# myscience/open-genie

Hardware: NVIDIA H100
Metric: videotokenizer_train_step_frames_per_sec (higher is better)
Workload: dtype bf16

## Files before the change

open_genie_b200/csrc/conv3d_igemm.cu:

```cuda
#include "og_host.cuh"
#include "og_ptx.cuh"

namespace og {
extern std::atomic<uint64_t> g_launches;

struct IgemmSeg {
  int cin_blocks;
  int n[3], tap0[3], tstep[3], sh0[3], shstep[3];
  int kh, kw;
};

struct IgemmParams {
  int nseg;
  IgemmSeg seg[2];
  int sx[3];
  int OT, OH, OW;
  int om[3], oo[3];
  int b_mn_major;
  int block_n;
  int num_n_tiles, num_m_tiles;
  int bw_log2, bh_log2, bt_log2, bn_log2;
  int tiles_w, tiles_h, tiles_t;
  int N, T, H, W;
  int n_out;
  long long ldo;
  void* out;
  int out_f32;
  int vec_ok;
  const float* bias0;
  const float* bias1;
  int num_stages;
  int num_kb;
  int fast_store;
  const __nv_bfloat16* residual;
  double* gn_sums;
  int splits;
  float* ws;
  long long ws_slab;
};


static constexpr int kBlockM = 128;
static constexpr int kBlockK = 64;
static constexpr int kABytes = kBlockM * kBlockK * 2;
static constexpr int kMaxStages = 8;
static constexpr int kThreads = 256;
static constexpr int kTailBytes = 256 + 1024 + 4 * 4096 + 256;
__host__ __device__ constexpr int acc_ld(int bn) { return bn + 4; }

template <int NV>
__device__ __forceinline__ void ld_acc_row(const float* src, uint32_t (&v)[32]) {
#pragma unroll
  for (int i = 0; i < NV / 4; ++i) {
    const float4 f = reinterpret_cast<const float4*>(src)[i];
    v[4 * i] = __float_as_uint(f.x);
    v[4 * i + 1] = __float_as_uint(f.y);
    v[4 * i + 2] = __float_as_uint(f.z);
    v[4 * i + 3] = __float_as_uint(f.w);
  }
#pragma unroll
  for (int i = NV; i < 32; ++i) v[i] = 0u;
}

struct TileCoord {
  int n0, t0, h0, w0;
};

__device__ __forceinline__ TileCoord decode_m_tile(const IgemmParams& p, int m_tile) {
  TileCoord c;
  int per_sample = p.tiles_w * p.tiles_h * p.tiles_t;
  const int tn = m_tile / per_sample;
  c.n0 = tn << p.bn_log2;
  int r = m_tile - tn * per_sample;
  int tw = r % p.tiles_w;
  r /= p.tiles_w;
  int th = r % p.tiles_h;
  int tt = r / p.tiles_h;
  c.w0 = tw << p.bw_log2;
  c.h0 = th << p.bh_log2;
  c.t0 = tt << p.bt_log2;
  return c;
}

template <int BN, int BMN>
__global__ void __launch_bounds__(kThreads, 1)
    og_conv_igemm_kernel(const __grid_constant__ CUtensorMap mapA0, const __grid_constant__ CUtensorMap mapA1,
                         const __grid_constant__ CUtensorMap mapB, const IgemmParams p) {
  extern __shared__ uint8_t smem_raw[];
  uint8_t* smem = reinterpret_cast<uint8_t*>((reinterpret_cast<uintptr_t>(smem_raw) + 1023) & ~uintptr_t(1023));
  const int b_bytes = p.block_n * kBlockK * 2;
  const int a_bytes = kABytes;
  const int stage_bytes = a_bytes + b_bytes;
  uint64_t* bars = reinterpret_cast<uint64_t*>(smem + p.num_stages * stage_bytes);
  uint64_t* full = bars;
  uint64_t* empty = bars + kMaxStages;
  float* bias_s = reinterpret_cast<float*>(bars + 32);
  uint8_t* stage_s = reinterpret_cast<uint8_t*>(bars + 32) + 1024;
  double* stat_s = reinterpret_cast<double*>(stage_s + 4 * 4096);
  float* acc_s = reinterpret_cast<float*>(reinterpret_cast<uint8_t*>(bars) + kTailBytes);

  const int warp = warp_idx_uniform();
  const int lane = threadIdx.x & 31;
  const int total_tiles = p.num_m_tiles * p.num_n_tiles * p.splits;

  if (warp == 0 && lane == 0) {
    tma_prefetch_desc(&mapA0);
    if (p.nseg > 1) tma_prefetch_desc(&mapA1);
    tma_prefetch_desc(&mapB);
    for (int s = 0; s < p.num_stages; ++s) {
      mbar_init(&full[s], 1);
      mbar_init(&empty[s], 4);
    }
    fence_mbar_init();
  }
  __syncthreads();

  if (warp == 0) {
    {
      int stage = 0;
      uint32_t phase = 0;
      for (int item = blockIdx.x; item < total_tiles; item += gridDim.x) {
        const int tile = item / p.splits, split = item - tile * p.splits;
        const int m_super = tile / p.num_n_tiles;
        const int n_tile = tile - m_super * p.num_n_tiles;
        const TileCoord tc = decode_m_tile(p, m_super);
        const int kb_begin = (int)(((long long)p.num_kb * split) / p.splits);
        const int kb_end = (int)(((long long)p.num_kb * (split + 1)) / p.splits);
        const int nkb0 = p.seg[0].cin_blocks * p.seg[0].n[0] * p.seg[0].n[1] * p.seg[0].n[2];
        int sidx = (kb_begin >= nkb0 && p.nseg > 1) ? 1 : 0;
        IgemmSeg sg = p.seg[sidx];
        int rel = kb_begin - (sidx ? nkb0 : 0);
        int tapc = rel / sg.cin_blocks;
        int cb = rel - tapc * sg.cin_blocks;
        int jt = tapc / (sg.n[1] * sg.n[2]);
        int jh = (tapc / sg.n[2]) % sg.n[1];
        int jw = tapc % sg.n[2];
        const int aw0 = tc.w0 * p.sx[2], ah0 = tc.h0 * p.sx[1], at0 = tc.t0 * p.sx[0];
        for (int kb = kb_begin; kb < kb_end; ++kb) {
          const CUtensorMap* mapA = (sidx == 0) ? &mapA0 : &mapA1;
          const int dt = sg.sh0[0] + jt * sg.shstep[0], dh = sg.sh0[1] + jh * sg.shstep[1],
                    dw = sg.sh0[2] + jw * sg.shstep[2];
          mbar_wait(&empty[stage], phase ^ 1);
          uint8_t* sa = smem + stage * stage_bytes;
          uint8_t* sb = sa + a_bytes;
          if (elect_one()) {
            mbar_expect_tx(&full[stage], (uint32_t)stage_bytes);
            tma_load_5d(sa, mapA, &full[stage], cb * kBlockK, aw0 + dw, ah0 + dh, at0 + dt, tc.n0);
            if (!BMN) {
              tma_load_2d(sb, &mapB, &full[stage], kb * kBlockK, n_tile * p.block_n);
            } else {
              const int tap = ((sg.tap0[0] + jt * sg.tstep[0]) * sg.kh + sg.tap0[1] + jh * sg.tstep[1]) * sg.kw +
                              sg.tap0[2] + jw * sg.tstep[2];
              for (int pp = 0; pp < p.block_n / 64; ++pp)
                tma_load_3d(sb + pp * (64 * 128), &mapB, &full[stage], n_tile * p.block_n + pp * 64, tap,
                            cb * kBlockK);
            }
          }
          __syncwarp();
          if (++stage == p.num_stages) {
            stage = 0;
            phase ^= 1;
          }
          if (++cb == sg.cin_blocks) {
            cb = 0;
            if (++jw == sg.n[2]) {
              jw = 0;
              if (++jh == sg.n[1]) {
                jh = 0;
                if (++jt == sg.n[0]) {
                  sidx = 1;
                  sg = p.seg[1];
                  jt = jh = jw = 0;
                }
              }
            }
          }
        }
      }
    }
  } else if (warp >= 4) {
    const int q = warp & 3;
    const int row = q * 32 + lane;
    const int et = threadIdx.x - 128;
    int stage = 0;
    uint32_t phase = 0;
    float fl_s = 0.f, fl_ss = 0.f;
    if (et == 0) stat_s[0] = stat_s[1] = 0.0;
    asm volatile("bar.sync 1, 128;" ::: "memory");
    for (int item = blockIdx.x; item < total_tiles; item += gridDim.x) {
      const int tile = item / p.splits;
      const int split = item - tile * p.splits;
      const int m_super = tile / p.num_n_tiles;
      const int n_tile = tile - m_super * p.num_n_tiles;
      const int nkb = (int)(((long long)p.num_kb * (split + 1)) / p.splits) -
                      (int)(((long long)p.num_kb * split) / p.splits);
      float acc[2][BN / 2];
#pragma unroll
      for (int hh = 0; hh < 2; ++hh)
#pragma unroll
        for (int i = 0; i < BN / 2; ++i) acc[hh][i] = 0.f;
      int prev = -1;
      for (int kb = 0; kb < nkb; ++kb) {
        mbar_wait(&full[stage], phase);
        const uint32_t a_addr = smem_u32(smem + stage * stage_bytes);
        const uint32_t b_addr = a_addr + a_bytes;
        wgmma_fence();
#pragma unroll
        for (int k = 0; k < kBlockK / 16; ++k) {
          const uint64_t bdesc = BMN ? gmma_desc_sw128(b_addr + k * 2048, 64 * 128, 1024)
                                     : gmma_desc_sw128(b_addr + k * 32, 16, 1024);
#pragma unroll
          for (int hh = 0; hh < 2; ++hh)
            wgmma_ss<BN, 0, BMN>(acc[hh], gmma_desc_sw128(a_addr + hh * 8192 + k * 32, 16, 1024), bdesc, 1);
        }
        wgmma_commit();
        wgmma_wait<1>();
        if (prev >= 0 && lane == 0) mbar_arrive(&empty[prev]);
        prev = stage;
        if (++stage == p.num_stages) {
          stage = 0;
          phase ^= 1;
        }
      }
      wgmma_wait<0>();
      reg_fence(acc[0]);
      reg_fence(acc[1]);
      if (prev >= 0 && lane == 0) mbar_arrive(&empty[prev]);
      asm volatile("bar.sync 1, 128;" ::: "memory");
      {
        const int r0 = q * 16 + (lane >> 2), c0 = 2 * (lane & 3);
#pragma unroll
        for (int hh = 0; hh < 2; ++hh)
#pragma unroll
          for (int j = 0; j < BN / 8; ++j) {
            float* d0 = acc_s + (hh * 64 + r0) * acc_ld(BN) + j * 8 + c0;
            *reinterpret_cast<float2*>(d0) = make_float2(acc[hh][4 * j], acc[hh][4 * j + 1]);
            *reinterpret_cast<float2*>(d0 + 8 * acc_ld(BN)) = make_float2(acc[hh][4 * j + 2], acc[hh][4 * j + 3]);
          }
      }
      asm volatile("bar.sync 1, 128;" ::: "memory");
      const float* acc_row = acc_s + row * acc_ld(BN);

      do {
      const TileCoord tc = decode_m_tile(p, m_super);
      const int dw = row & ((1 << p.bw_log2) - 1);
      const int dh = (row >> p.bw_log2) & ((1 << p.bh_log2) - 1);
      const int dt = (row >> (p.bw_log2 + p.bh_log2)) & ((1 << p.bt_log2) - 1);
      const int dn = row >> (p.bw_log2 + p.bh_log2 + p.bt_log2);
      const int vn = tc.n0 + dn, vt = tc.t0 + dt, vh = tc.h0 + dh, vw = tc.w0 + dw;
      const bool row_ok = vn < p.N && vt < p.T && vh < p.H && vw < p.W;
      const long long vox = (((long long)vn * p.OT + vt * p.om[0] + p.oo[0]) * p.OH + vh * p.om[1] + p.oo[1]) * p.OW +
                            vw * p.om[2] + p.oo[2];
      const int col0 = n_tile * p.block_n;

      if (p.splits > 1) {
        for (int c = 0; c < p.block_n; c += 32) {
          if (col0 + c >= p.n_out) break;
          uint32_t v[32];
          ld_acc_row<32>(acc_row + c, v);
          if (row_ok) {
            float* dst = p.ws + (long long)split * p.ws_slab + vox * p.ldo + col0 + c;
            if (p.vec_ok && col0 + c + 32 <= p.n_out) {
#pragma unroll
              for (int j = 0; j < 32; j += 4)
                __stcg(reinterpret_cast<float4*>(dst + j),
                       make_float4(__uint_as_float(v[j]), __uint_as_float(v[j + 1]), __uint_as_float(v[j + 2]),
                                   __uint_as_float(v[j + 3])));
            } else {
              for (int j = 0; j < 32; ++j)
                if (col0 + c + j < p.n_out) dst[j] = __uint_as_float(v[j]);
            }
          }
        }
        continue;
      }

      if (p.fast_store) {
        {
          asm volatile("bar.sync 1, 128;" ::: "memory");
          for (int j = et; j < p.block_n; j += 128) {
            const int col = col0 + j;
            float b = 0.f;
            if (col < p.n_out) {
              if (p.bias0) b += __ldg(p.bias0 + col);
              if (p.bias1) b += __ldg(p.bias1 + col);
            }
            bias_s[j] = b;
          }
          asm volatile("bar.sync 1, 128;" ::: "memory");
        }
        float st_s = 0.f, st_ss = 0.f;
        uint8_t* my_stage = stage_s + q * 4096;
        __nv_bfloat16* outp = reinterpret_cast<__nv_bfloat16*>(p.out);
        for (int c = 0; c < p.block_n; c += 64) {
          if (col0 + c >= p.n_out) break;
          uint32_t v0[32], v1[32];
          ld_acc_row<32>(acc_row + c, v0);
          ld_acc_row<32>(acc_row + c + 32, v1);
          if (p.residual && row_ok) {
            const uint4* rp = reinterpret_cast<const uint4*>(p.residual + vox * p.ldo + col0 + c);
#pragma unroll
            for (int j = 0; j < 8; ++j) {
              const uint4 u = __ldg(rp + j);
              const __nv_bfloat162* hh = reinterpret_cast<const __nv_bfloat162*>(&u);
#pragma unroll
              for (int e = 0; e < 4; ++e) {
                const float2 f = __bfloat1622float2(hh[e]);
                uint32_t* dst = (j < 4) ? &v0[8 * j + 2 * e] : &v1[8 * (j - 4) + 2 * e];
                dst[0] = __float_as_uint(__uint_as_float(dst[0]) + f.x);
                dst[1] = __float_as_uint(__uint_as_float(dst[1]) + f.y);
              }
            }
          }
#pragma unroll
          for (int j = 0; j < 32; ++j) {
            v0[j] = __float_as_uint(__uint_as_float(v0[j]) + bias_s[c + j]);
            v1[j] = __float_as_uint(__uint_as_float(v1[j]) + bias_s[c + 32 + j]);
          }
          if (p.gn_sums && row_ok) {
#pragma unroll
            for (int j = 0; j < 32; ++j) {
              const float r0 = __bfloat162float(__float2bfloat16_rn(__uint_as_float(v0[j])));
              const float r1 = __bfloat162float(__float2bfloat16_rn(__uint_as_float(v1[j])));
              st_s += r0 + r1;
              st_ss = fmaf(r0, r0, fmaf(r1, r1, st_ss));
            }
          }
#pragma unroll
          for (int j = 0; j < 4; ++j) {
            uint4 u;
            u.x = pack_bf16x2(__uint_as_float(v0[8 * j + 0]), __uint_as_float(v0[8 * j + 1]));
            u.y = pack_bf16x2(__uint_as_float(v0[8 * j + 2]), __uint_as_float(v0[8 * j + 3]));
            u.z = pack_bf16x2(__uint_as_float(v0[8 * j + 4]), __uint_as_float(v0[8 * j + 5]));
            u.w = pack_bf16x2(__uint_as_float(v0[8 * j + 6]), __uint_as_float(v0[8 * j + 7]));
            *reinterpret_cast<uint4*>(my_stage + lane * 128 + ((j ^ (lane & 7)) << 4)) = u;
          }
#pragma unroll
          for (int j = 0; j < 4; ++j) {
            uint4 u;
            u.x = pack_bf16x2(__uint_as_float(v1[8 * j + 0]), __uint_as_float(v1[8 * j + 1]));
            u.y = pack_bf16x2(__uint_as_float(v1[8 * j + 2]), __uint_as_float(v1[8 * j + 3]));
            u.z = pack_bf16x2(__uint_as_float(v1[8 * j + 4]), __uint_as_float(v1[8 * j + 5]));
            u.w = pack_bf16x2(__uint_as_float(v1[8 * j + 6]), __uint_as_float(v1[8 * j + 7]));
            *reinterpret_cast<uint4*>(my_stage + lane * 128 + (((j + 4) ^ (lane & 7)) << 4)) = u;
          }
          __syncwarp();
          const int chunk = lane & 7;
#pragma unroll
          for (int i = 0; i < 8; ++i) {
            const int r = i * 4 + (lane >> 3);
            const long long rvox = __shfl_sync(0xffffffffu, vox, r);
            const int rok = __shfl_sync(0xffffffffu, (int)row_ok, r);
            const uint4 u = *reinterpret_cast<const uint4*>(my_stage + r * 128 + ((chunk ^ (r & 7)) << 4));
            if (rok) *reinterpret_cast<uint4*>(outp + rvox * p.ldo + col0 + c + chunk * 8) = u;
          }
          __syncwarp();
        }
        fl_s += st_s;
        fl_ss += st_ss;
        continue;
      }

      for (int c = 0; c < p.block_n; c += 32) {
        uint32_t v[32];
        if (BN >= 32)
          ld_acc_row<32>(acc_row + c, v);
        else
          ld_acc_row<16>(acc_row + c, v);
        const int cbase = col0 + c;
        if (cbase >= p.n_out || !row_ok) continue;
        float f[32];
#pragma unroll
        for (int j = 0; j < 32; ++j) {
          float b = 0.f;
          const int col = cbase + j;
          if (col < p.n_out) {
            if (p.bias0) b += __ldg(p.bias0 + col);
            if (p.bias1) b += __ldg(p.bias1 + col);
          }
          f[j] = __uint_as_float(v[j]) + b;
          if (p.residual && col < p.n_out && row_ok) f[j] += __bfloat162float(p.residual[vox * p.ldo + col]);
        }
        if (p.out_f32) {
          float* o = reinterpret_cast<float*>(p.out) + vox * p.ldo + cbase;
          if (p.vec_ok && cbase + 32 <= p.n_out) {
#pragma unroll
            for (int j = 0; j < 32; j += 4)
              *reinterpret_cast<float4*>(o + j) = make_float4(f[j], f[j + 1], f[j + 2], f[j + 3]);
          } else {
            for (int j = 0; j < 32; ++j)
              if (cbase + j < p.n_out) o[j] = f[j];
          }
        } else {
          __nv_bfloat16* o = reinterpret_cast<__nv_bfloat16*>(p.out) + vox * p.ldo + cbase;
          if (p.vec_ok && cbase + 32 <= p.n_out) {
#pragma unroll
            for (int j = 0; j < 32; j += 8) {
              uint4 u;
              u.x = pack_bf16x2(f[j], f[j + 1]);
              u.y = pack_bf16x2(f[j + 2], f[j + 3]);
              u.z = pack_bf16x2(f[j + 4], f[j + 5]);
              u.w = pack_bf16x2(f[j + 6], f[j + 7]);
              *reinterpret_cast<uint4*>(o + j) = u;
            }
          } else {
            for (int j = 0; j < 32; ++j)
              if (cbase + j < p.n_out) o[j] = __float2bfloat16_rn(f[j]);
          }
        }
      }
      } while (0);
      if (p.fast_store && p.splits == 1 && p.gn_sums) {
        const TileCoord tcf = decode_m_tile(p, m_super);
        for (int o = 16; o > 0; o >>= 1) {
          fl_s += __shfl_xor_sync(0xffffffffu, fl_s, o);
          fl_ss += __shfl_xor_sync(0xffffffffu, fl_ss, o);
        }
        if (lane == 0) {
          atomicAdd(&stat_s[0], (double)fl_s);
          atomicAdd(&stat_s[1], (double)fl_ss);
        }
        asm volatile("bar.sync 1, 128;" ::: "memory");
        if (et == 0) {
          atomicAdd(&p.gn_sums[(long long)tcf.n0 * 2], stat_s[0]);
          atomicAdd(&p.gn_sums[(long long)tcf.n0 * 2 + 1], stat_s[1]);
          stat_s[0] = 0.0;
          stat_s[1] = 0.0;
        }
        fl_s = fl_ss = 0.f;
      }
    }
  }
}

template <int VEC>
__global__ void __launch_bounds__(256)
    og_splitk_finish_kernel(const float* __restrict__ ws, long long slab, int nslab, const float* __restrict__ bias0,
                            const float* __restrict__ bias1, void* __restrict__ out, int out_f32, int n_out,
                            long long per_sample, double* __restrict__ gn_sums) {
  const long long base = (long long)blockIdx.y * per_sample;
  float s = 0.f, ss = 0.f;
  for (long long i = ((long long)blockIdx.x * blockDim.x + threadIdx.x) * VEC; i < per_sample;
       i += (long long)gridDim.x * blockDim.x * VEC) {
    float v[VEC];
    if (VEC == 4) {
      const float4 a = __ldcg(reinterpret_cast<const float4*>(ws + base + i));
      v[0] = a.x; v[1 % VEC] = a.y; v[2 % VEC] = a.z; v[3 % VEC] = a.w;
      for (int k = 1; k < nslab; ++k) {
        const float4 b = __ldcg(reinterpret_cast<const float4*>(ws + (long long)k * slab + base + i));
        v[0] += b.x; v[1 % VEC] += b.y; v[2 % VEC] += b.z; v[3 % VEC] += b.w;
      }
    } else {
      v[0] = __ldcg(ws + base + i);
      for (int k = 1; k < nslab; ++k) v[0] += __ldcg(ws + (long long)k * slab + base + i);
    }
    const int col = (int)(i % n_out);
#pragma unroll
    for (int e = 0; e < VEC; ++e) {
      if (bias0) v[e] += __ldg(bias0 + col + e);
      if (bias1) v[e] += __ldg(bias1 + col + e);
    }
    if (out_f32) {
#pragma unroll
      for (int e = 0; e < VEC; ++e) reinterpret_cast<float*>(out)[base + i + e] = v[e];
    } else {
      __nv_bfloat16 h[VEC];
#pragma unroll
      for (int e = 0; e < VEC; ++e) {
        h[e] = __float2bfloat16_rn(v[e]);
        const float r = __bfloat162float(h[e]);
        s += r;
        ss = fmaf(r, r, ss);
      }
      __nv_bfloat16* o = reinterpret_cast<__nv_bfloat16*>(out) + base + i;
      if (VEC == 4)
        *reinterpret_cast<uint2*>(o) = *reinterpret_cast<const uint2*>(h);
      else
        o[0] = h[0];
    }
  }
  if (gn_sums) {
    __shared__ float red[2][8];
#pragma unroll
    for (int off = 16; off >= 1; off >>= 1) {
      s += __shfl_xor_sync(0xffffffffu, s, off);
      ss += __shfl_xor_sync(0xffffffffu, ss, off);
    }
    if ((threadIdx.x & 31) == 0) {
      red[0][threadIdx.x >> 5] = s;
      red[1][threadIdx.x >> 5] = ss;
    }
    __syncthreads();
    if (threadIdx.x == 0) {
      double a = 0.0, b = 0.0;
      for (int w = 0; w < (int)(blockDim.x >> 5); ++w) {
        a += (double)red[0][w];
        b += (double)red[1][w];
      }
      atomicAdd(gn_sums + 2 * blockIdx.y, a);
      atomicAdd(gn_sums + 2 * blockIdx.y + 1, b);
    }
  }
}

static int pick_block_n(int n_out, bool mn_major) {
  int bn = 16;
  while (bn < n_out && bn < 128) bn *= 2;
  if (mn_major && bn < 64) bn = 64;
  return bn;
}

template <int BN, int BMN>
static int launch_igemm_kernel(int grid, size_t smem_bytes, cudaStream_t stream, const CUtensorMap& mapA0,
                               const CUtensorMap& mapA1, const CUtensorMap& mapB, const IgemmParams& p) {
  static bool attr_set = false;
  if (!attr_set) {
    OG_CHECK_CUDA(cudaFuncSetAttribute(og_conv_igemm_kernel<BN, BMN>, cudaFuncAttributeMaxDynamicSharedMemorySize,
                                       227 * 1024));
    attr_set = true;
  }
  og_conv_igemm_kernel<BN, BMN><<<grid, kThreads, smem_bytes, stream>>>(mapA0, mapA1, mapB, p);
  OG_CHECK_CUDA(cudaGetLastError());
  return OG_OK;
}

struct IgemmLaunch {
  const void* a0 = nullptr;
  int c0 = 0;
  int aT = 0, aH = 0, aW = 0;
  int astride[3] = {1, 1, 1};
  const void* a1 = nullptr;
  int c1 = 0;
  IgemmSeg segs[2];
  int nseg = 1;
  const void* w = nullptr;
  int ldw = 0, k_off = 0, b_mn_major = 0, b_rows = 0, b_ntaps = 0;
  const float* bias0 = nullptr;
  const float* bias1 = nullptr;
  const void* residual = nullptr;
  void* out = nullptr;
  int out_f32 = 0;
  int N = 0, T = 0, H = 0, W = 0;
  int OT = 0, OH = 0, OW = 0;
  int om[3] = {1, 1, 1}, oo[3] = {0, 0, 0};
  int n_out = 0;
  void* workspace = nullptr;
  size_t workspace_bytes = 0;
  double* gn_sums = nullptr;
};

static IgemmSeg make_seg(int cin_blocks, int kt, int kh, int kw, int pt, int ph, int pw, int sgn) {
  IgemmSeg g;
  g.cin_blocks = cin_blocks;
  const int k[3] = {kt, kh, kw}, pd[3] = {pt, ph, pw};
  for (int d = 0; d < 3; ++d) {
    g.n[d] = k[d];
    g.tap0[d] = 0;
    g.tstep[d] = 1;
    g.sh0[d] = -sgn * pd[d];
    g.shstep[d] = sgn;
  }
  g.kh = kh;
  g.kw = kw;
  return g;
}

static int launch_igemm(const IgemmLaunch& L, cudaStream_t stream) {
  const int N = L.N, T = L.T, H = L.H, W = L.W, n_out = L.n_out;
  OG_REQUIRE(N > 0 && T > 0 && H > 0 && W > 0 && n_out > 0, "conv3d: empty problem");
  const bool plain = (L.OT == 0) && L.astride[0] == 1 && L.astride[1] == 1 && L.astride[2] == 1;
  int bw, bh, bt, bn;
  choose_voxel_box(kBlockM, N, T, H, W, &bw, &bh, &bt, &bn);
  IgemmParams p;
  memset(&p, 0, sizeof(p));
  p.nseg = L.nseg;
  p.num_kb = 0;
  for (int s = 0; s < L.nseg; ++s) {
    p.seg[s] = L.segs[s];
    p.num_kb += L.segs[s].cin_blocks * L.segs[s].n[0] * L.segs[s].n[1] * L.segs[s].n[2];
  }
  OG_REQUIRE(p.num_kb > 0, "conv3d: empty reduction");
  for (int d = 0; d < 3; ++d) {
    p.sx[d] = L.astride[d];
    p.om[d] = L.om[d];
    p.oo[d] = L.oo[d];
  }
  p.OT = L.OT ? L.OT : T;
  p.OH = L.OH ? L.OH : H;
  p.OW = L.OW ? L.OW : W;
  p.b_mn_major = L.b_mn_major;
  p.bw_log2 = ilog2(bw);
  p.bh_log2 = ilog2(bh);
  p.bt_log2 = ilog2(bt);
  p.bn_log2 = ilog2(bn);
  p.tiles_w = (W + bw - 1) / bw;
  p.tiles_h = (H + bh - 1) / bh;
  p.tiles_t = (T + bt - 1) / bt;
  p.N = N;
  p.T = T;
  p.H = H;
  p.W = W;
  p.num_m_tiles = ((N + bn - 1) / bn) * p.tiles_w * p.tiles_h * p.tiles_t;
  p.block_n = pick_block_n(n_out, L.b_mn_major != 0);
  p.num_n_tiles = (n_out + p.block_n - 1) / p.block_n;
  p.n_out = n_out;
  p.ldo = n_out;
  p.out = L.out;
  p.out_f32 = L.out_f32;
  p.vec_ok = L.out_f32 ? (n_out % 4 == 0) : (n_out % 8 == 0);
  p.bias0 = L.bias0;
  p.bias1 = L.bias1;
  p.residual = reinterpret_cast<const __nv_bfloat16*>(L.residual);
  const int stage_bytes = kABytes + p.block_n * kBlockK * 2;
  p.fast_store = (!L.out_f32 && n_out % 64 == 0 && p.block_n % 64 == 0) ? 1 : 0;
  p.splits = 1;
  if (plain) {
    const long long tiles = (long long)p.num_m_tiles * p.num_n_tiles;
    const size_t need = (size_t)N * T * H * W * n_out * sizeof(float);
    if (tiles * 2 <= num_sms() && p.num_kb >= 32 && L.workspace && !L.residual) {
      int sp = (int)(num_sms() / tiles);
      if (sp > p.num_kb / 8) sp = p.num_kb / 8;
      if (sp > 16) sp = 16;
      if ((size_t)sp > L.workspace_bytes / need) sp = (int)(L.workspace_bytes / need);
      if (sp >= 2) {
        p.splits = sp;
        p.ws = reinterpret_cast<float*>(L.workspace);
        p.ws_slab = (long long)(need / sizeof(float));
      }
    }
  }
  const int tail_bytes = kTailBytes + kBlockM * acc_ld(p.block_n) * 4 ;
  int stages = (227 * 1024 - 1024  - tail_bytes) / stage_bytes;
  if (stages > kMaxStages) stages = kMaxStages;
  p.num_stages = stages;
  const size_t smem_bytes = (size_t)stages * stage_bytes + 1024 + tail_bytes;

  CUtensorMap mapA0, mapA1, mapB;
  {
    const int c0 = L.c0;
    const int st = L.astride[0], sh = L.astride[1], sw = L.astride[2];
    uint64_t dims[5] = {(uint64_t)c0, (uint64_t)L.aW, (uint64_t)L.aH, (uint64_t)L.aT, (uint64_t)N};
    uint64_t str[4] = {(uint64_t)c0 * 2, (uint64_t)L.aW * c0 * 2, (uint64_t)L.aH * L.aW * c0 * 2,
                       (uint64_t)L.aT * L.aH * L.aW * c0 * 2};
    uint32_t box[5] = {kBlockK, (uint32_t)(bw * sw), (uint32_t)(bh * sh), (uint32_t)(bt * st), (uint32_t)bn};
    uint32_t es[5] = {1, (uint32_t)sw, (uint32_t)sh, (uint32_t)st, 1};
    OG_REQUIRE(box[1] <= 256 && box[2] <= 256 && box[3] <= 256, "conv3d: strided box exceeds the TMA limit");
    int r = make_tmap_bf16(&mapA0, L.a0, 5, dims, str, box, es);
    if (r != OG_OK) return r;
  }
  if (L.nseg > 1) {
    const int c1 = L.c1;
    uint64_t dims[5] = {(uint64_t)c1, (uint64_t)W, (uint64_t)H, (uint64_t)T, (uint64_t)N};
    uint64_t str[4] = {(uint64_t)c1 * 2, (uint64_t)W * c1 * 2, (uint64_t)H * W * c1 * 2, (uint64_t)T * H * W * c1 * 2};
    uint32_t box[5] = {kBlockK, (uint32_t)bw, (uint32_t)bh, (uint32_t)bt, (uint32_t)bn};
    int r = make_tmap_bf16(&mapA1, L.a1, 5, dims, str, box);
    if (r != OG_OK) return r;
  } else {
    mapA1 = mapA0;
  }
  const __nv_bfloat16* wb = reinterpret_cast<const __nv_bfloat16*>(L.w) + L.k_off;
  if (!L.b_mn_major) {
    uint64_t ktot = (uint64_t)p.num_kb * kBlockK;
    uint64_t dims[2] = {ktot, (uint64_t)n_out};
    uint64_t str[1] = {(uint64_t)L.ldw * 2};
    uint32_t box[2] = {kBlockK, (uint32_t)p.block_n};
    int r = make_tmap_bf16(&mapB, wb, 2, dims, str, box);
    if (r != OG_OK) return r;
  } else {
    uint64_t dims[3] = {(uint64_t)n_out, (uint64_t)L.b_ntaps, (uint64_t)L.b_rows};
    uint64_t str[2] = {(uint64_t)n_out * 2, (uint64_t)L.ldw * 2};
    uint32_t box[3] = {64, 1, 64};
    int r = make_tmap_bf16(&mapB, wb, 3, dims, str, box);
    if (r != OG_OK) return r;
  }

  const bool can_fuse = plain && p.fast_store && p.splits == 1 && bn == 1 && n_out <= 65536;
  p.gn_sums = (L.gn_sums && can_fuse) ? L.gn_sums : nullptr;
  const int total_tiles = p.num_m_tiles * p.num_n_tiles * p.splits;
  int grid = num_sms();
  if (grid > total_tiles) grid = total_tiles;
  int rc;
  switch (p.block_n * 2 + p.b_mn_major) {
    case 16 * 2: rc = launch_igemm_kernel<16, 0>(grid, smem_bytes, stream, mapA0, mapA1, mapB, p); break;
    case 32 * 2: rc = launch_igemm_kernel<32, 0>(grid, smem_bytes, stream, mapA0, mapA1, mapB, p); break;
    case 64 * 2: rc = launch_igemm_kernel<64, 0>(grid, smem_bytes, stream, mapA0, mapA1, mapB, p); break;
    case 128 * 2: rc = launch_igemm_kernel<128, 0>(grid, smem_bytes, stream, mapA0, mapA1, mapB, p); break;
    case 64 * 2 + 1: rc = launch_igemm_kernel<64, 1>(grid, smem_bytes, stream, mapA0, mapA1, mapB, p); break;
    case 128 * 2 + 1: rc = launch_igemm_kernel<128, 1>(grid, smem_bytes, stream, mapA0, mapA1, mapB, p); break;
    default: OG_REQUIRE(false, "conv3d: no kernel for block_n=%d", p.block_n);
  }
  if (rc != OG_OK) return rc;
  g_launches.fetch_add(1);
  bool finish_did_stats = false;
  if (p.splits > 1) {
    const long long per_sample = (long long)T * H * W * n_out;
    finish_did_stats = L.gn_sums && !L.out_f32;
    double* gs = finish_did_stats ? L.gn_sums : nullptr;
    const int vec = (n_out % 4 == 0) ? 4 : 1;
    long long bx = (per_sample / vec + 255) / 256;
    const long long cap = ((long long)num_sms() * 8 + N - 1) / N;
    if (bx > cap) bx = cap;
    if (bx < 1) bx = 1;
    dim3 grid((unsigned)bx, (unsigned)N);
    if (vec == 4)
      og_splitk_finish_kernel<4><<<grid, 256, 0, stream>>>(p.ws, p.ws_slab, p.splits, L.bias0, L.bias1, L.out, L.out_f32,
                                                            n_out, per_sample, gs);
    else
      og_splitk_finish_kernel<1><<<grid, 256, 0, stream>>>(p.ws, p.ws_slab, p.splits, L.bias0, L.bias1, L.out, L.out_f32,
                                                            n_out, per_sample, gs);
    OG_CHECK_CUDA(cudaGetLastError());
    g_launches.fetch_add(1);
  }
  if (L.gn_sums && !p.gn_sums && !finish_did_stats) {
    OG_REQUIRE(!L.out_f32 && plain, "conv3d: GroupNorm statistics need a plain bf16 output");
    int r = og_gn_stats(L.out, N, (int64_t)T * H * W, n_out, 1, L.gn_sums, (og_stream_t)stream);
    if (r != OG_OK) return r;
  }
  return OG_OK;
}

}

extern "C" int og_conv3d_fwd(const void* x0, int c0, int kt, int kh, int kw, int pt, int ph, int pw, const void* x1,
                             int c1, const void* w, int ldw, const float* bias0, const float* bias1,
                             const void* residual, void* out, int out_f32, int N, int T, int H, int W, int cout,
                             void* workspace, size_t workspace_bytes, double* gn_sums, og_stream_t stream) {
  using namespace og;
  OG_REQUIRE(x0 && w && out, "conv3d_fwd: null pointer");
  OG_REQUIRE(c0 > 0 && c0 % 64 == 0, "conv3d_fwd: c0=%d must be a positive multiple of 64", c0);
  OG_REQUIRE(!x1 || (c1 > 0 && c1 % 64 == 0), "conv3d_fwd: c1=%d must be a multiple of 64", c1);
  OG_REQUIRE(kt >= 1 && kh >= 1 && kw >= 1 && pt >= 0 && ph >= 0 && pw >= 0 && pt < kt && ph < kh && pw < kw,
             "conv3d_fwd: bad kernel/padding (%d,%d,%d)/(%d,%d,%d)", kt, kh, kw, pt, ph, pw);
  const int ktot = kt * kh * kw * c0 + (x1 ? c1 : 0);
  OG_REQUIRE(ldw >= ktot && ldw % 8 == 0, "conv3d_fwd: ldw=%d must be >= %d and a multiple of 8", ldw, ktot);
  IgemmLaunch L;
  L.a0 = x0; L.c0 = c0; L.aT = T; L.aH = H; L.aW = W;
  L.a1 = x1; L.c1 = c1;
  L.segs[0] = make_seg(c0 / 64, kt, kh, kw, pt, ph, pw, +1);
  L.segs[1] = make_seg(c1 / 64, 1, 1, 1, 0, 0, 0, +1);
  L.nseg = x1 ? 2 : 1;
  L.w = w; L.ldw = ldw;
  L.bias0 = bias0; L.bias1 = bias1; L.residual = residual;
  L.out = out; L.out_f32 = out_f32;
  L.N = N; L.T = T; L.H = H; L.W = W; L.n_out = cout;
  L.workspace = workspace; L.workspace_bytes = workspace_bytes;
  L.gn_sums = gn_sums;
  return launch_igemm(L, (cudaStream_t)stream);
}

extern "C" int og_conv3d_dgrad(const void* dy, int cout, int w_rows, const void* w, int ldw, int k_off, int kt, int kh,
                               int kw, int pt, int ph, int pw, void* dx, int dx_f32, int N, int T, int H, int W,
                               int cin, void* workspace, size_t workspace_bytes, og_stream_t stream) {
  using namespace og;
  OG_REQUIRE(dy && w && dx, "conv3d_dgrad: null pointer");
  OG_REQUIRE(cout > 0 && cout % 64 == 0, "conv3d_dgrad: cout=%d must be a multiple of 64", cout);
  OG_REQUIRE(cin > 0 && cin % 64 == 0, "conv3d_dgrad: cin=%d must be a multiple of 64", cin);
  OG_REQUIRE(k_off % 8 == 0 && ldw % 8 == 0, "conv3d_dgrad: k_off/ldw must be multiples of 8");
  OG_REQUIRE(w_rows > 0 && w_rows <= cout, "conv3d_dgrad: w_rows=%d must be in (0, cout]", w_rows);
  IgemmLaunch L;
  L.a0 = dy; L.c0 = cout; L.aT = T; L.aH = H; L.aW = W;
  L.segs[0] = make_seg(cout / 64, kt, kh, kw, pt, ph, pw, -1);
  L.nseg = 1;
  L.w = w; L.ldw = ldw; L.k_off = k_off; L.b_mn_major = 1; L.b_rows = w_rows; L.b_ntaps = kt * kh * kw;
  L.out = dx; L.out_f32 = dx_f32;
  L.N = N; L.T = T; L.H = H; L.W = W; L.n_out = cin;
  L.workspace = workspace; L.workspace_bytes = workspace_bytes;
  return launch_igemm(L, (cudaStream_t)stream);
}

static int out_extent(int in, int pad_front, int pad_back, int k, int s) { return (in + pad_front + pad_back - k) / s + 1; }

extern "C" int og_conv3d_strided_fwd(const void* x, int cin, int kt, int kh, int kw, int st, int sh, int sw, int pt, int ph,
                                     int pw, const void* w, int ldw, const float* bias, void* out, int out_f32, int N, int T,
                                     int H, int W, int cout, og_stream_t stream) {
  using namespace og;
  OG_REQUIRE(x && w && out, "conv3d_strided_fwd: null pointer");
  OG_REQUIRE(cin > 0 && cin % 64 == 0, "conv3d_strided_fwd: cin=%d must be a positive multiple of 64", cin);
  OG_REQUIRE(kt >= 1 && kh >= 1 && kw >= 1 && st >= 1 && sh >= 1 && sw >= 1 && st <= 8 && sh <= 8 && sw <= 8 && pt >= 0 &&
                 ph >= 0 && pw >= 0, "conv3d_strided_fwd: bad kernel / stride / padding");
  OG_REQUIRE(ldw >= kt * kh * kw * cin && ldw % 8 == 0, "conv3d_strided_fwd: bad ldw=%d", ldw);
  const int To = out_extent(T, pt, 0, kt, st), Ho = out_extent(H, ph, ph, kh, sh), Wo = out_extent(W, pw, pw, kw, sw);
  OG_REQUIRE(To >= 1 && Ho >= 1 && Wo >= 1, "conv3d_strided_fwd: empty output");
  IgemmLaunch L;
  L.a0 = x; L.c0 = cin; L.aT = T; L.aH = H; L.aW = W;
  L.astride[0] = st; L.astride[1] = sh; L.astride[2] = sw;
  L.segs[0] = make_seg(cin / 64, kt, kh, kw, pt, ph, pw, +1);
  L.nseg = 1;
  L.w = w; L.ldw = ldw;
  L.bias0 = bias;
  L.out = out; L.out_f32 = out_f32;
  L.N = N; L.T = To; L.H = Ho; L.W = Wo; L.n_out = cout;
  return launch_igemm(L, (cudaStream_t)stream);
}

extern "C" int og_conv3d_strided_dgrad(const void* dy, int cout, int w_rows, const void* w, int ldw, int kt, int kh, int kw,
                                       int st, int sh, int sw, int pt, int ph, int pw, void* dx, int N, int T, int H, int W,
                                       int cin, og_stream_t stream) {
  using namespace og;
  OG_REQUIRE(dy && w && dx, "conv3d_strided_dgrad: null pointer");
  OG_REQUIRE(cout > 0 && cout % 64 == 0 && cin > 0 && cin % 64 == 0, "conv3d_strided_dgrad: channels must be multiples of 64");
  OG_REQUIRE(w_rows > 0 && w_rows <= cout && ldw % 8 == 0, "conv3d_strided_dgrad: bad w_rows / ldw");
  const int To = out_extent(T, pt, 0, kt, st), Ho = out_extent(H, ph, ph, kh, sh), Wo = out_extent(W, pw, pw, kw, sw);
  OG_REQUIRE(To >= 1 && Ho >= 1 && Wo >= 1, "conv3d_strided_dgrad: empty output");
  const int k[3] = {kt, kh, kw}, s[3] = {st, sh, sw}, pd[3] = {pt, ph, pw}, in[3] = {T, H, W};
  bool any_empty = false;
  for (int d = 0; d < 3; ++d)
    if (k[d] < s[d]) any_empty = true;
  if (any_empty) OG_CHECK_CUDA(cudaMemsetAsync(dx, 0, (size_t)N * T * H * W * cin * 2, (cudaStream_t)stream));
  for (int ct = 0; ct < st; ++ct)
    for (int ch = 0; ch < sh; ++ch)
      for (int cw = 0; cw < sw; ++cw) {
        const int cls[3] = {ct, ch, cw};
        IgemmLaunch L;
        L.segs[0].cin_blocks = cout / 64;
        L.segs[0].kh = kh;
        L.segs[0].kw = kw;
        int grid[3];
        bool empty = false;
        for (int d = 0; d < 3; ++d) {
          const int r = ((cls[d] - pd[d]) % s[d] + s[d]) % s[d];
          const int ntap = cls[d] < k[d] ? (k[d] - 1 - cls[d]) / s[d] + 1 : 0;
          grid[d] = in[d] > r ? (in[d] - r + s[d] - 1) / s[d] : 0;
          if (ntap == 0 || grid[d] == 0) empty = true;
          L.segs[0].n[d] = ntap;
          L.segs[0].tap0[d] = cls[d];
          L.segs[0].tstep[d] = s[d];
          L.segs[0].sh0[d] = (r + pd[d] - cls[d]) / s[d];
          L.segs[0].shstep[d] = -1;
          L.om[d] = s[d];
          L.oo[d] = r;
        }
        if (empty) continue;
        L.a0 = dy; L.c0 = cout; L.aT = To; L.aH = Ho; L.aW = Wo;
        L.nseg = 1;
        L.w = w; L.ldw = ldw; L.b_mn_major = 1; L.b_rows = w_rows; L.b_ntaps = kt * kh * kw;
        L.out = dx; L.out_f32 = 0;
        L.N = N; L.T = grid[0]; L.H = grid[1]; L.W = grid[2]; L.n_out = cin;
        L.OT = T; L.OH = H; L.OW = W;
        int rc = launch_igemm(L, (cudaStream_t)stream);
        if (rc != OG_OK) return rc;
      }
  return OG_OK;
}
```

Measured before the change: 958.0.

## Ping-pong two consumer warpgroups with register-direct epilogue in conv igemm

```diff
diff --git a/open_genie_b200/csrc/conv3d_igemm.cu b/open_genie_b200/csrc/conv3d_igemm.cu
--- a/open_genie_b200/csrc/conv3d_igemm.cu
+++ b/open_genie_b200/csrc/conv3d_igemm.cu
@@ -43,24 +43,11 @@
 static constexpr int kBlockM = 128;
 static constexpr int kBlockK = 64;
 static constexpr int kABytes = kBlockM * kBlockK * 2;
-static constexpr int kMaxStages = 8;
-static constexpr int kThreads = 256;
-static constexpr int kTailBytes = 256 + 1024 + 4 * 4096 + 256;
-__host__ __device__ constexpr int acc_ld(int bn) { return bn + 4; }
-
-template <int NV>
-__device__ __forceinline__ void ld_acc_row(const float* src, uint32_t (&v)[32]) {
-#pragma unroll
-  for (int i = 0; i < NV / 4; ++i) {
-    const float4 f = reinterpret_cast<const float4*>(src)[i];
-    v[4 * i] = __float_as_uint(f.x);
-    v[4 * i + 1] = __float_as_uint(f.y);
-    v[4 * i + 2] = __float_as_uint(f.z);
-    v[4 * i + 3] = __float_as_uint(f.w);
-  }
-#pragma unroll
-  for (int i = NV; i < 32; ++i) v[i] = 0u;
-}
+static constexpr int kMaxStages = 4;
+static constexpr int kThreads = 384;
+static constexpr int kConsumerTail = 512 + 4 * 4096 + 64 + 128 * 8;
+static constexpr int kTailBytes = 256 + 2 * kConsumerTail;
+static constexpr int kOrderBar = 3;
 
 struct TileCoord {
   int n0, t0, h0, w0;
@@ -82,6 +69,32 @@
   return c;
 }
 
+__device__ __forceinline__ bool tile_row(const IgemmParams& p, const TileCoord& tc, int row, long long& vox) {
+  const int dw = row & ((1 << p.bw_log2) - 1);
+  const int dh = (row >> p.bw_log2) & ((1 << p.bh_log2) - 1);
+  const int dt = (row >> (p.bw_log2 + p.bh_log2)) & ((1 << p.bt_log2) - 1);
+  const int dn = row >> (p.bw_log2 + p.bh_log2 + p.bt_log2);
+  const int vn = tc.n0 + dn, vt = tc.t0 + dt, vh = tc.h0 + dh, vw = tc.w0 + dw;
+  vox = (((long long)vn * p.OT + vt * p.om[0] + p.oo[0]) * p.OH + vh * p.om[1] + p.oo[1]) * p.OW + vw * p.om[2] + p.oo[2];
+  return vn < p.N && vt < p.T && vh < p.H && vw < p.W;
+}
+
+__device__ __forceinline__ float bias_at(const IgemmParams& p, int col) {
+  float b = 0.f;
+  if (col < p.n_out) {
+    if (p.bias0) b += __ldg(p.bias0 + col);
+    if (p.bias1) b += __ldg(p.bias1 + col);
+  }
+  return b;
+}
+
+__device__ __forceinline__ void named_bar_sync(int id, int count) {
+  asm volatile("bar.sync %0, %1;" ::"r"(id), "r"(count) : "memory");
+}
+__device__ __forceinline__ void named_bar_arrive(int id, int count) {
+  asm volatile("bar.arrive %0, %1;" ::"r"(id), "r"(count) : "memory");
+}
+
 template <int BN, int BMN>
 __global__ void __launch_bounds__(kThreads, 1)
     og_conv_igemm_kernel(const __grid_constant__ CUtensorMap mapA0, const __grid_constant__ CUtensorMap mapA1,
@@ -94,10 +107,6 @@
   uint64_t* bars = reinterpret_cast<uint64_t*>(smem + p.num_stages * stage_bytes);
   uint64_t* full = bars;
   uint64_t* empty = bars + kMaxStages;
-  float* bias_s = reinterpret_cast<float*>(bars + 32);
-  uint8_t* stage_s = reinterpret_cast<uint8_t*>(bars + 32) + 1024;
-  double* stat_s = reinterpret_cast<double*>(stage_s + 4 * 4096);
-  float* acc_s = reinterpret_cast<float*>(reinterpret_cast<uint8_t*>(bars) + kTailBytes);
 
   const int warp = warp_idx_uniform();
   const int lane = threadIdx.x & 31;
@@ -115,8 +124,9 @@
   }
   __syncthreads();
 
-  if (warp == 0) {
-    {
+  if (warp < 4) {
+    asm volatile("setmaxnreg.dec.sync.aligned.u32 40;");
+    if (warp == 0) {
       int stage = 0;
       uint32_t phase = 0;
       for (int item = blockIdx.x; item < total_tiles; item += gridDim.x) {
@@ -178,27 +188,44 @@
         }
       }
     }
-  } else if (warp >= 4) {
+  } else {
+    asm volatile("setmaxnreg.inc.sync.aligned.u32 232;");
+    const int wg = (warp >> 2) - 1;
     const int q = warp & 3;
-    const int row = q * 32 + lane;
-    const int et = threadIdx.x - 128;
+    const int et = threadIdx.x - 128 * (wg + 1);
+    const int epi_bar = 1 + wg;
+    uint8_t* tail = reinterpret_cast<uint8_t*>(bars) + 256 + wg * kConsumerTail;
+    float* bias_s = reinterpret_cast<float*>(tail);
+    uint8_t* my_stage = tail + 512 + q * 4096;
+    double* stat_s = reinterpret_cast<double*>(tail + 512 + 4 * 4096);
+    float2* row_s = reinterpret_cast<float2*>(tail + 512 + 4 * 4096 + 64);
+    const int cl = 2 * (lane & 3);
     int stage = 0;
     uint32_t phase = 0;
     float fl_s = 0.f, fl_ss = 0.f;
     if (et == 0) stat_s[0] = stat_s[1] = 0.0;
-    asm volatile("bar.sync 1, 128;" ::: "memory");
-    for (int item = blockIdx.x; item < total_tiles; item += gridDim.x) {
+    named_bar_sync(epi_bar, 128);
+    int i = 0;
+    for (int item = blockIdx.x; item < total_tiles; item += gridDim.x, ++i) {
       const int tile = item / p.splits;
       const int split = item - tile * p.splits;
+      const int nkb = (int)(((long long)p.num_kb * (split + 1)) / p.splits) -
+                      (int)(((long long)p.num_kb * split) / p.splits);
+      if ((i & 1) != wg) {
+        stage += nkb;
+        const int wraps = stage / p.num_stages;
+        stage -= wraps * p.num_stages;
+        phase ^= wraps & 1;
+        continue;
+      }
       const int m_super = tile / p.num_n_tiles;
       const int n_tile = tile - m_super * p.num_n_tiles;
-      const int nkb = (int)(((long long)p.num_kb * (split + 1)) / p.splits) -
-                      (int)(((long long)p.num_kb * split) / p.splits);
+      if (i > 0) named_bar_sync(kOrderBar + wg, 256);
       float acc[2][BN / 2];
 #pragma unroll
       for (int hh = 0; hh < 2; ++hh)
 #pragma unroll
-        for (int i = 0; i < BN / 2; ++i) acc[hh][i] = 0.f;
+        for (int j = 0; j < BN / 2; ++j) acc[hh][j] = 0.f;
       int prev = -1;
       for (int kb = 0; kb < nkb; ++kb) {
         mbar_wait(&full[stage], phase);
@@ -222,212 +249,166 @@
           phase ^= 1;
         }
       }
+      if (item + gridDim.x < total_tiles) named_bar_arrive(kOrderBar + (wg ^ 1), 256);
       wgmma_wait<0>();
       reg_fence(acc[0]);
       reg_fence(acc[1]);
-      if (prev >= 0 && lane == 0) mbar_arrive(&empty[prev]);
-      asm volatile("bar.sync 1, 128;" ::: "memory");
-      {
-        const int r0 = q * 16 + (lane >> 2), c0 = 2 * (lane & 3);
+      if (lane == 0) mbar_arrive(&empty[prev]);
+
+      const TileCoord tc = decode_m_tile(p, m_super);
+      const int col0 = n_tile * p.block_n;
+      if (p.splits > 1) {
+        float* ws = p.ws + (long long)split * p.ws_slab + col0;
 #pragma unroll
         for (int hh = 0; hh < 2; ++hh)
 #pragma unroll
-          for (int j = 0; j < BN / 8; ++j) {
-            float* d0 = acc_s + (hh * 64 + r0) * acc_ld(BN) + j * 8 + c0;
-            *reinterpret_cast<float2*>(d0) = make_float2(acc[hh][4 * j], acc[hh][4 * j + 1]);
-            *reinterpret_cast<float2*>(d0 + 8 * acc_ld(BN)) = make_float2(acc[hh][4 * j + 2], acc[hh][4 * j + 3]);
-          }
-      }
-      asm volatile("bar.sync 1, 128;" ::: "memory");
-      const float* acc_row = acc_s + row * acc_ld(BN);
-
-      do {
-      const TileCoord tc = decode_m_tile(p, m_super);
-      const int dw = row & ((1 << p.bw_log2) - 1);
-      const int dh = (row >> p.bw_log2) & ((1 << p.bh_log2) - 1);
-      const int dt = (row >> (p.bw_log2 + p.bh_log2)) & ((1 << p.bt_log2) - 1);
-      const int dn = row >> (p.bw_log2 + p.bh_log2 + p.bt_log2);
-      const int vn = tc.n0 + dn, vt = tc.t0 + dt, vh = tc.h0 + dh, vw = tc.w0 + dw;
-      const bool row_ok = vn < p.N && vt < p.T && vh < p.H && vw < p.W;
-      const long long vox = (((long long)vn * p.OT + vt * p.om[0] + p.oo[0]) * p.OH + vh * p.om[1] + p.oo[1]) * p.OW +
-                            vw * p.om[2] + p.oo[2];
-      const int col0 = n_tile * p.block_n;
-
-      if (p.splits > 1) {
-        for (int c = 0; c < p.block_n; c += 32) {
-          if (col0 + c >= p.n_out) break;
-          uint32_t v[32];
-          ld_acc_row<32>(acc_row + c, v);
-          if (row_ok) {
-            float* dst = p.ws + (long long)split * p.ws_slab + vox * p.ldo + col0 + c;
-            if (p.vec_ok && col0 + c + 32 <= p.n_out) {
-#pragma unroll
-              for (int j = 0; j < 32; j += 4)
-                __stcg(reinterpret_cast<float4*>(dst + j),
-                       make_float4(__uint_as_float(v[j]), __uint_as_float(v[j + 1]), __uint_as_float(v[j + 2]),
-                                   __uint_as_float(v[j + 3])));
-            } else {
-              for (int j = 0; j < 32; ++j)
-                if (col0 + c + j < p.n_out) dst[j] = __uint_as_float(v[j]);
-            }
-          }
-        }
-        continue;
-      }
-
-      if (p.fast_store) {
-        {
-          asm volatile("bar.sync 1, 128;" ::: "memory");
-          for (int j = et; j < p.block_n; j += 128) {
-            const int col = col0 + j;
-            float b = 0.f;
-            if (col < p.n_out) {
-              if (p.bias0) b += __ldg(p.bias0 + col);
-              if (p.bias1) b += __ldg(p.bias1 + col);
-            }
-            bias_s[j] = b;
-          }
-          asm volatile("bar.sync 1, 128;" ::: "memory");
-        }
-        float st_s = 0.f, st_ss = 0.f;
-        uint8_t* my_stage = stage_s + q * 4096;
-        __nv_bfloat16* outp = reinterpret_cast<__nv_bfloat16*>(p.out);
-        for (int c = 0; c < p.block_n; c += 64) {
-          if (col0 + c >= p.n_out) break;
-          uint32_t v0[32], v1[32];
-          ld_acc_row<32>(acc_row + c, v0);
-          ld_acc_row<32>(acc_row + c + 32, v1);
-          if (p.residual && row_ok) {
-            const uint4* rp = reinterpret_cast<const uint4*>(p.residual + vox * p.ldo + col0 + c);
-#pragma unroll
-            for (int j = 0; j < 8; ++j) {
-              const uint4 u = __ldg(rp + j);
-              const __nv_bfloat162* hh = reinterpret_cast<const __nv_bfloat162*>(&u);
-#pragma unroll
-              for (int e = 0; e < 4; ++e) {
-                const float2 f = __bfloat1622float2(hh[e]);
-                uint32_t* dst = (j < 4) ? &v0[8 * j + 2 * e] : &v1[8 * (j - 4) + 2 * e];
-                dst[0] = __float_as_uint(__uint_as_float(dst[0]) + f.x);
-                dst[1] = __float_as_uint(__uint_as_float(dst[1]) + f.y);
+          for (int h8 = 0; h8 < 2; ++h8) {
+            long long vox;
+            if (!tile_row(p, tc, hh * 64 + q * 16 + (lane >> 2) + 8 * h8, vox)) continue;
+            float* dst = ws + vox * p.ldo;
+#pragma unroll
+            for (int j = 0; j < BN / 8; ++j) {
+              const int col = col0 + 8 * j + cl;
+              const float v0 = acc[hh][4 * j + 2 * h8], v1 = acc[hh][4 * j + 2 * h8 + 1];
+              if (p.vec_ok && col + 1 < p.n_out) {
+                __stcg(reinterpret_cast<float2*>(dst + 8 * j + cl), make_float2(v0, v1));
+              } else {
+                if (col < p.n_out) dst[8 * j + cl] = v0;
+                if (col + 1 < p.n_out) dst[8 * j + cl + 1] = v1;
               }
             }
           }
-#pragma unroll
-          for (int j = 0; j < 32; ++j) {
-            v0[j] = __float_as_uint(__uint_as_float(v0[j]) + bias_s[c + j]);
-            v1[j] = __float_as_uint(__uint_as_float(v1[j]) + bias_s[c + 32 + j]);
-          }
-          if (p.gn_sums && row_ok) {
-#pragma unroll
-            for (int j = 0; j < 32; ++j) {
-              const float r0 = __bfloat162float(__float2bfloat16_rn(__uint_as_float(v0[j])));
-              const float r1 = __bfloat162float(__float2bfloat16_rn(__uint_as_float(v1[j])));
-              st_s += r0 + r1;
-              st_ss = fmaf(r0, r0, fmaf(r1, r1, st_ss));
+      } else if (p.fast_store) {
+        named_bar_sync(epi_bar, 128);
+        for (int j = et; j < p.block_n; j += 128) bias_s[j] = bias_at(p, col0 + j);
+        named_bar_sync(epi_bar, 128);
+        long long my_vox;
+        const int my_ok = tile_row(p, tc, (lane >> 4) * 64 + q * 16 + (lane & 15), my_vox);
+        __nv_bfloat16* outp = reinterpret_cast<__nv_bfloat16*>(p.out) + col0;
+        const __nv_bfloat16* resp = p.residual + col0;
+        const int chunk = lane & 7;
+#pragma unroll
+        for (int c = 0; c < BN; c += 64) {
+          if (col0 + c >= p.n_out) break;
+          if (p.residual) {
+#pragma unroll
+            for (int it = 0; it < 8; ++it) {
+              const int r = it * 4 + (lane >> 3);
+              const long long rvox = __shfl_sync(0xffffffffu, my_vox, r);
+              const int rok = __shfl_sync(0xffffffffu, my_ok, r);
+              uint4 u = make_uint4(0u, 0u, 0u, 0u);
+              if (rok) u = __ldg(reinterpret_cast<const uint4*>(resp + rvox * p.ldo + c + chunk * 8));
+              *reinterpret_cast<uint4*>(my_stage + r * 128 + ((chunk ^ (r & 7)) << 4)) = u;
             }
-          }
-#pragma unroll
-          for (int j = 0; j < 4; ++j) {
-            uint4 u;
-            u.x = pack_bf16x2(__uint_as_float(v0[8 * j + 0]), __uint_as_float(v0[8 * j + 1]));
-            u.y = pack_bf16x2(__uint_as_float(v0[8 * j + 2]), __uint_as_float(v0[8 * j + 3]));
-            u.z = pack_bf16x2(__uint_as_float(v0[8 * j + 4]), __uint_as_float(v0[8 * j + 5]));
-            u.w = pack_bf16x2(__uint_as_float(v0[8 * j + 6]), __uint_as_float(v0[8 * j + 7]));
-            *reinterpret_cast<uint4*>(my_stage + lane * 128 + ((j ^ (lane & 7)) << 4)) = u;
-          }
-#pragma unroll
-          for (int j = 0; j < 4; ++j) {
-            uint4 u;
-            u.x = pack_bf16x2(__uint_as_float(v1[8 * j + 0]), __uint_as_float(v1[8 * j + 1]));
-            u.y = pack_bf16x2(__uint_as_float(v1[8 * j + 2]), __uint_as_float(v1[8 * j + 3]));
-            u.z = pack_bf16x2(__uint_as_float(v1[8 * j + 4]), __uint_as_float(v1[8 * j + 5]));
-            u.w = pack_bf16x2(__uint_as_float(v1[8 * j + 6]), __uint_as_float(v1[8 * j + 7]));
-            *reinterpret_cast<uint4*>(my_stage + lane * 128 + (((j + 4) ^ (lane & 7)) << 4)) = u;
-          }
+            __syncwarp();
+          }
+#pragma unroll
+          for (int hh = 0; hh < 2; ++hh)
+#pragma unroll
+            for (int h8 = 0; h8 < 2; ++h8) {
+              const int lr = hh * 16 + h8 * 8 + (lane >> 2);
+#pragma unroll
+              for (int jj = 0; jj < 8; ++jj) {
+                const int j = c / 8 + jj;
+                uint32_t* w = reinterpret_cast<uint32_t*>(my_stage + lr * 128 + ((jj ^ (lane >> 2)) << 4)) + (lane & 3);
+                float v0 = acc[hh][4 * j + 2 * h8], v1 = acc[hh][4 * j + 2 * h8 + 1];
+                if (p.residual) {
+                  const float2 r = __bfloat1622float2(*reinterpret_cast<const __nv_bfloat162*>(w));
+                  v0 += r.x;
+                  v1 += r.y;
+                }
+                const float2 b = *reinterpret_cast<const float2*>(bias_s + c + 8 * jj + cl);
+                *w = pack_bf16x2(v0 + b.x, v1 + b.y);
+              }
+            }
           __syncwarp();
-          const int chunk = lane & 7;
-#pragma unroll
-          for (int i = 0; i < 8; ++i) {
-            const int r = i * 4 + (lane >> 3);
-            const long long rvox = __shfl_sync(0xffffffffu, vox, r);
-            const int rok = __shfl_sync(0xffffffffu, (int)row_ok, r);
+          if (p.gn_sums && my_ok) {
+#pragma unroll
+            for (int jc = 0; jc < 4; ++jc) {
+              const uint4 u0 = *reinterpret_cast<const uint4*>(my_stage + lane * 128 + ((jc ^ (lane & 7)) << 4));
+              const uint4 u1 = *reinterpret_cast<const uint4*>(my_stage + lane * 128 + (((jc + 4) ^ (lane & 7)) << 4));
+              const __nv_bfloat162* h0 = reinterpret_cast<const __nv_bfloat162*>(&u0);
+              const __nv_bfloat162* h1 = reinterpret_cast<const __nv_bfloat162*>(&u1);
+#pragma unroll
+              for (int e = 0; e < 4; ++e) {
+                const float2 f0 = __bfloat1622float2(h0[e]), f1 = __bfloat1622float2(h1[e]);
+                fl_s += f0.x + f1.x;
+                fl_ss = fmaf(f0.x, f0.x, fmaf(f1.x, f1.x, fl_ss));
+                fl_s += f0.y + f1.y;
+                fl_ss = fmaf(f0.y, f0.y, fmaf(f1.y, f1.y, fl_ss));
+              }
+            }
+          }
+#pragma unroll
+          for (int it = 0; it < 8; ++it) {
+            const int r = it * 4 + (lane >> 3);
+            const long long rvox = __shfl_sync(0xffffffffu, my_vox, r);
+            const int rok = __shfl_sync(0xffffffffu, my_ok, r);
             const uint4 u = *reinterpret_cast<const uint4*>(my_stage + r * 128 + ((chunk ^ (r & 7)) << 4));
-            if (rok) *reinterpret_cast<uint4*>(outp + rvox * p.ldo + col0 + c + chunk * 8) = u;
+            if (rok) *reinterpret_cast<uint4*>(outp + rvox * p.ldo + c + chunk * 8) = u;
           }
           __syncwarp();
         }
-        fl_s += st_s;
-        fl_ss += st_ss;
-        continue;
-      }
-
-      for (int c = 0; c < p.block_n; c += 32) {
-        uint32_t v[32];
-        if (BN >= 32)
-          ld_acc_row<32>(acc_row + c, v);
-        else
-          ld_acc_row<16>(acc_row + c, v);
-        const int cbase = col0 + c;
-        if (cbase >= p.n_out || !row_ok) continue;
-        float f[32];
-#pragma unroll
-        for (int j = 0; j < 32; ++j) {
-          float b = 0.f;
-          const int col = cbase + j;
-          if (col < p.n_out) {
-            if (p.bias0) b += __ldg(p.bias0 + col);
-            if (p.bias1) b += __ldg(p.bias1 + col);
-          }
-          f[j] = __uint_as_float(v[j]) + b;
-          if (p.residual && col < p.n_out && row_ok) f[j] += __bfloat162float(p.residual[vox * p.ldo + col]);
+        if (p.gn_sums) {
+          row_s[(lane >> 4) * 64 + q * 16 + (lane & 15)] = make_float2(fl_s, fl_ss);
+          named_bar_sync(epi_bar, 128);
+          const float2 rs = row_s[q * 32 + lane];
+          fl_s = rs.x;
+          fl_ss = rs.y;
+          for (int o = 16; o > 0; o >>= 1) {
+            fl_s += __shfl_xor_sync(0xffffffffu, fl_s, o);
+            fl_ss += __shfl_xor_sync(0xffffffffu, fl_ss, o);
+          }
+          if (lane == 0) {
+            atomicAdd(&stat_s[0], (double)fl_s);
+            atomicAdd(&stat_s[1], (double)fl_ss);
+          }
+          named_bar_sync(epi_bar, 128);
+          if (et == 0) {
+            atomicAdd(&p.gn_sums[(long long)tc.n0 * 2], stat_s[0]);
+            atomicAdd(&p.gn_sums[(long long)tc.n0 * 2 + 1], stat_s[1]);
+            stat_s[0] = 0.0;
+            stat_s[1] = 0.0;
+          }
+          fl_s = fl_ss = 0.f;
         }
-        if (p.out_f32) {
-          float* o = reinterpret_cast<float*>(p.out) + vox * p.ldo + cbase;
-          if (p.vec_ok && cbase + 32 <= p.n_out) {
-#pragma unroll
-            for (int j = 0; j < 32; j += 4)
-              *reinterpret_cast<float4*>(o + j) = make_float4(f[j], f[j + 1], f[j + 2], f[j + 3]);
-          } else {
-            for (int j = 0; j < 32; ++j)
-              if (cbase + j < p.n_out) o[j] = f[j];
-          }
-        } else {
-          __nv_bfloat16* o = reinterpret_cast<__nv_bfloat16*>(p.out) + vox * p.ldo + cbase;
-          if (p.vec_ok && cbase + 32 <= p.n_out) {
-#pragma unroll
-            for (int j = 0; j < 32; j += 8) {
-              uint4 u;
-              u.x = pack_bf16x2(f[j], f[j + 1]);
-              u.y = pack_bf16x2(f[j + 2], f[j + 3]);
-              u.z = pack_bf16x2(f[j + 4], f[j + 5]);
-              u.w = pack_bf16x2(f[j + 6], f[j + 7]);
-              *reinterpret_cast<uint4*>(o + j) = u;
+      } else {
+#pragma unroll
+        for (int hh = 0; hh < 2; ++hh)
+#pragma unroll
+          for (int h8 = 0; h8 < 2; ++h8) {
+            long long vox;
+            if (!tile_row(p, tc, hh * 64 + q * 16 + (lane >> 2) + 8 * h8, vox)) continue;
+#pragma unroll
+            for (int j = 0; j < BN / 8; ++j) {
+              const int col = col0 + 8 * j + cl;
+              if (col >= p.n_out) continue;
+              const bool two = col + 1 < p.n_out;
+              float f0 = acc[hh][4 * j + 2 * h8] + bias_at(p, col);
+              float f1 = acc[hh][4 * j + 2 * h8 + 1] + bias_at(p, col + 1);
+              if (p.residual) {
+                f0 += __bfloat162float(p.residual[vox * p.ldo + col]);
+                if (two) f1 += __bfloat162float(p.residual[vox * p.ldo + col + 1]);
+              }
+              if (p.out_f32) {
+                float* o = reinterpret_cast<float*>(p.out) + vox * p.ldo + col;
+                if (p.vec_ok && two) {
+                  *reinterpret_cast<float2*>(o) = make_float2(f0, f1);
+                } else {
+                  o[0] = f0;
+                  if (two) o[1] = f1;
+                }
+              } else {
+                __nv_bfloat16* o = reinterpret_cast<__nv_bfloat16*>(p.out) + vox * p.ldo + col;
+                if (p.vec_ok && two) {
+                  *reinterpret_cast<uint32_t*>(o) = pack_bf16x2(f0, f1);
+                } else {
+                  o[0] = __float2bfloat16_rn(f0);
+                  if (two) o[1] = __float2bfloat16_rn(f1);
+                }
+              }
             }
-          } else {
-            for (int j = 0; j < 32; ++j)
-              if (cbase + j < p.n_out) o[j] = __float2bfloat16_rn(f[j]);
-          }
-        }
-      }
-      } while (0);
-      if (p.fast_store && p.splits == 1 && p.gn_sums) {
-        const TileCoord tcf = decode_m_tile(p, m_super);
-        for (int o = 16; o > 0; o >>= 1) {
-          fl_s += __shfl_xor_sync(0xffffffffu, fl_s, o);
-          fl_ss += __shfl_xor_sync(0xffffffffu, fl_ss, o);
-        }
-        if (lane == 0) {
-          atomicAdd(&stat_s[0], (double)fl_s);
-          atomicAdd(&stat_s[1], (double)fl_ss);
-        }
-        asm volatile("bar.sync 1, 128;" ::: "memory");
-        if (et == 0) {
-          atomicAdd(&p.gn_sums[(long long)tcf.n0 * 2], stat_s[0]);
-          atomicAdd(&p.gn_sums[(long long)tcf.n0 * 2 + 1], stat_s[1]);
-          stat_s[0] = 0.0;
-          stat_s[1] = 0.0;
-        }
-        fl_s = fl_ss = 0.f;
+          }
       }
     }
   }
@@ -629,11 +610,10 @@
       }
     }
   }
-  const int tail_bytes = kTailBytes + kBlockM * acc_ld(p.block_n) * 4 ;
-  int stages = (227 * 1024 - 1024  - tail_bytes) / stage_bytes;
+  int stages = (227 * 1024 - 1024  - kTailBytes) / stage_bytes;
   if (stages > kMaxStages) stages = kMaxStages;
   p.num_stages = stages;
-  const size_t smem_bytes = (size_t)stages * stage_bytes + 1024 + tail_bytes;
+  const size_t smem_bytes = (size_t)stages * stage_bytes + 1024 + kTailBytes;
 
   CUtensorMap mapA0, mapA1, mapB;
   {
```

After: 988.7 (median of 6 runs). +3.2%, better.
